# NeRdTheNed/deft4j

Measured on NVIDIA B200. Metric: input MB/s optimised (-m NONE), higher is better.
Workload: dtype u8

## Files before the change

deft4j_b200/csrc/engine.cuh:

```cuda
#pragma once
#include "enum.cuh"
#include "parse.cuh"

namespace d4 {

#ifndef D4_ENG_NT
#define D4_ENG_NT 256
#endif
#ifndef D4_ENG_MINB
#define D4_ENG_MINB 4
#endif
constexpr int ENG_NT = D4_ENG_NT;
constexpr int ENG_NW = ENG_NT / 32;
constexpr int ERR_TREE = 11, ERR_ROUNDS = 12, ERR_WRITER = 2, ERR_POOL = 15, ERR_INTERNAL = 16;

__device__ long long* g_trace = nullptr;
__device__ unsigned g_trace_cap = 0;
__device__ unsigned g_trace_n = 0;

struct Cand {
    Tab tab;
    Hdr hdr;
    long long payload;
    uint16_t mid, tabid;
    uint32_t pad2;
};
__device__ __forceinline__ long long cand_size(const Cand& c) { return c.payload + (c.tab.type == 2 ? c.hdr.bits : 0); }

struct BlkView {
    const uint32_t* sym;
    const uint32_t* symout;
    const uint8_t* out;
    uint32_t n;
    uint32_t nwords;
    uint64_t ulen;
    uint64_t out_off;
};

constexpr int DC_TILE = 512;
constexpr int DCN = 16;
constexpr int LCN = 12;
constexpr int MAXLIT = 64;
constexpr int WS_BYTES = 3072;
#ifndef D4_HQS
#define D4_HQS 4608
#endif
constexpr int HQS = D4_HQS, HQL = 1024;
constexpr int SLOT_B = MAXM, SLOT_BEST = MAXM + 1;
static_assert(DC_TILE == 32 * 16 && DC_TILE > 258, "a tile is one warp-wide 128-bit load and no match spans more than two tiles");

#ifdef D4_PROF
__device__ unsigned long long g_prof[64];
#define P0() const long long p0_ = clock64()
#define P1(cat) do { if (threadIdx.x == 0) { atomicAdd(&g_prof[cat], (unsigned long long)(clock64() - p0_)); atomicAdd(&g_prof[32 + (cat)], 1ull); } } while (0)
#define PCOUNT(cat, k) do { if (threadIdx.x == 0) atomicAdd(&g_prof[32 + (cat)], (unsigned long long)(k)); } while (0)
#else
#define P0()
#define P1(cat)
#define PCOUNT(cat, k)
#endif
enum { PR_BLOCK = 0, PR_ROUND, PR_SWEEP, PR_SELECT, PR_PASS, PR_DC, PR_RECODE, PR_TREES, PR_HDR_DEFAULT, PR_HDROP, PR_TRIALS,
       PR_LOAD, PR_MATERIAL, PR_REBASE, PR_INTERN_MASK, PR_INTERN_TAB, PR_FIXED, PR_SLOWTREE, PR_SEGMENTED, PR_HIST,
       PR_PASS_MAIN, PR_PASS_HQ, PR_LEAST_APPLY, PR_PASS_LEAST, PR_MASKS };

struct EngSmem {
    SymState sym;
// ... 16 lines not shown
    int sweepOk[4], segImproved, segmentedRound;
    struct { long long bestSize, restMin; SC best; unsigned bestIndex, candIndex; int bestStored, bestArg; } carry;
    unsigned char tabDc[MAXT];
    unsigned short dcOwner[DCN];
    int dcNext;
    unsigned char tabLit[MAXT];
    unsigned long long litHash[MAXLIT];
    unsigned short litRep[MAXLIT];
    unsigned char litSlot[MAXLIT];
    unsigned char slotLit[LCN];
    int nLit, litNext;
    uint32_t ctab[256];
    uint8_t refL[32], refD[32];
    union alignas(16) {
        unsigned char ws[ENG_NW][WS_BYTES];
        uint32_t P[ENG_NW][DC_TILE + 4 + 36];
        struct { Tab tab; Hdr hdr; TreeWsCL ws; } mat;
        struct { uint32_t nS, nL; uint32_t qs[HQS]; uint32_t ql[HQL]; } hq;
    } u;
};

__shared__ EngSmem g_es;
#define ES (&g_es)

struct EngScratch {
    unsigned char* slab;
    size_t stride;
    size_t oMasks;
    size_t oTabs;
    size_t oHdrs;
    size_t oHists;
    size_t oTabHash;
    size_t oDc;
    size_t oKd;
    size_t oMinfo;
    size_t oTileFirst;
    size_t oTrialAll;
    size_t oRecs;
    size_t oSlowWs;
    size_t oPerm;
    size_t oDcBits;
    size_t oItems;
    uint32_t maxwords, maxtiles;
};
inline size_t eng_scratch_layout(EngScratch& sc, uint32_t maxwords, uint64_t maxu) {
    sc.maxwords = maxwords;
    sc.maxtiles = (uint32_t)(maxu / DC_TILE + 4);
    const size_t maxn = (size_t)maxwords * 32;
    size_t o = 0;
    auto take = [&](size_t bytes) { const size_t at = o; o = (o + bytes + 255) & ~(size_t)255; return at; };
    sc.oRecs = take(2 * sizeof(Cand));
    sc.oTabHash = take(sizeof(unsigned long long) * MAXT);
    sc.oTabs = take(sizeof(Tab) * (MAXT + ENG_NW));
    sc.oTileFirst = take(4 * (size_t)sc.maxtiles);
    sc.oMinfo = take(4 * maxn);
    sc.oPerm = take(4 * maxn);
    sc.oItems = take(4 * ((size_t)maxwords + 64));
    sc.oDc = take(2 * maxn * LCN);
    sc.oKd = take(2 * maxn);
    sc.oDcBits = take(4 * (size_t)maxwords * 2 * DCN);
    sc.oMasks = take(4 * (size_t)(MAXM + 2) * maxwords);
    sc.oHists = take(4 * (size_t)(MAXM + 2) * 320);
    sc.oHdrs = take(sizeof(Hdr) * MAXH);
    sc.oTrialAll = take(4 * (size_t)MAXT * 56);
    sc.oSlowWs = take(sizeof(TreeWs<290, 584>) * ENG_NW);
    sc.stride = (o + ((size_t)2 << 20) - 1) & ~(((size_t)2 << 20) - 1);
    return sc.stride;
}

struct Eng {
    static constexpr short DC_BLOCKED = 0x7FFF, DC_NOT_MATCH = 0x7FFE;
    BlkView v;
    uint32_t* masks;
    uint32_t maxwords, maxn;
    Tab* tabs;
    Hdr* hdrs;
    uint32_t* hists;
    unsigned long long* tabHash;
    short* dc;
    uint16_t* kd;
    uint32_t* minfo;
    uint32_t* tileFirst;
    int* trialAll;
    Cand* recs;
    TreeWs<290, 584>* slowWs;
    uint32_t* perm;
    uint32_t* dcBits;
    uint32_t* items;
    int tid;
    bool bigWeights;

    __device__ uint32_t* maskp(int id) const { return masks + (size_t)id * maxwords; }
    __device__ uint32_t* histp(int id) const { return hists + (size_t)id * 320; }

    __device__ __noinline__ unsigned long long hash_words(const uint32_t* p, int nwords32) {
        unsigned long long h = 0;
#pragma unroll 1
        for (int k = tid; k < nwords32; k += ENG_NT) {
            unsigned long long x = (unsigned long long)p[k] + 0x9E3779B97F4A7C15ull * (unsigned long long)(k + 1);
            x ^= x >> 30; x *= 0xBF58476D1CE4E5B9ull; x ^= x >> 27; x *= 0x94D049BB133111EBull; x ^= x >> 31;
            h += x;
        }
#pragma unroll 1
        for (int d = 16; d > 0; d >>= 1) h += __shfl_xor_sync(0xffffffffu, h, d);
        if ((tid & 31) == 0) ES->hred[tid >> 5] = h;
        __syncthreads();
        unsigned long long r = 0;
#pragma unroll 1
        for (int k = 0; k < ENG_NW; k++) r += ES->hred[k];
        __syncthreads();
        return r | 1ull;
    }
    static __device__ __forceinline__ unsigned long long hash_words_warp(const uint32_t* p, int nwords32, int lane) {
        unsigned long long h = 0;
// ... 69 lines not shown
    }

    __device__ __noinline__ int intern_mask(unsigned long long h) {
        P0();
        const int fresh = ES->sym.nMasks;
        const uint32_t* q = maskp(fresh);
        __syncthreads();
        if (tid == 0) { ES->tmpIdx = -1; ES->redAny2 = 0; }
        __syncthreads();
#pragma unroll 1
        for (int k = tid; k < fresh; k += ENG_NT)
            if (ES->maskHash[k] == h) atomicMax(&ES->tmpIdx, k);
        __syncthreads();
        int hit = ES->tmpIdx;
        if (hit >= 0) {
            const uint32_t* a = maskp(hit);
            bool diff = false;
#pragma unroll 1
            for (uint32_t k = tid; k < v.nwords; k += ENG_NT) diff |= a[k] != q[k];
            if (diff) ES->redAny2 = 1;
            __syncthreads();
            if (ES->redAny2) hit = -1;
        }
        __syncthreads();
        if (hit < 0) {
            hit = fresh;
            if (tid == 0) { ES->maskHash[fresh] = h; ES->sym.rc[fresh].state = ST_EMPTY; ES->sym.nMasks = fresh + 1; }
        }
        __syncthreads();
        P1(PR_INTERN_MASK);
        return hit;
    }

    __device__ __noinline__ void build_views() {
        const uint32_t a0 = (uint32_t)(v.out_off & ~15ull);
        const uint32_t ntiles = (uint32_t)(((v.out_off - a0) + v.ulen) / DC_TILE) + 2;
#pragma unroll 1
        for (uint32_t t = tid; t < ntiles; t += ENG_NT) tileFirst[t] = v.n;
        __syncthreads();
#pragma unroll 1
        for (uint32_t i = tid; i < v.n; i += ENG_NT) {
            const uint32_t s = v.sym[i];
            const uint32_t rel = v.symout[i] - a0;
            const bool mt = sym_is_match(s);
            const uint32_t kq = mt ? (uint32_t)(sym_lensym(s) - 256) : 0u;
            const uint32_t dsy = mt ? (uint32_t)dist_sym(sym_dist(s)) : 0u;
            minfo[i] = mt ? ((s & 0x1FF) | (dsy << 9) | (kq << 14) | ((rel & (DC_TILE - 1)) << 19)) : 0u;
            kd[i] = (uint16_t)(kq | (dsy << 5));
            const uint32_t ti = rel / DC_TILE;
            const int tprev = i ? (int)((v.symout[i - 1] - a0) / DC_TILE) : -1;
            if ((int)ti != tprev) tileFirst[ti] = i;
        }
        if (tid < 32) ES->leastCnt[tid] = 0;
        __syncthreads();
#pragma unroll 1
        for (uint32_t i = tid; i < v.n; i += ENG_NT) { const uint32_t s = v.sym[i]; if (sym_is_match(s)) atomicAdd(&ES->leastCnt[sym_lensym(s) - 257], 1); }
        __syncthreads();
        if (tid == 0) {
            uint32_t acc = 0;
#pragma unroll 1
            for (int b = 0; b < 32; b++) { ES->binStart[b] = acc; acc += (uint32_t)ES->leastCnt[b]; ES->leastCnt[b] = (int)ES->binStart[b]; }
            ES->binStart[32] = acc;
        }
        __syncthreads();
        if (tid == 0) {
            uint32_t acc = 0;
#pragma unroll 1
            for (int b = 0; b < 32; b++) { ES->itemStart[b] = acc; acc += (ES->binStart[b + 1] - ES->binStart[b] + 31) / 32; }
            ES->itemStart[32] = acc;
        }
#pragma unroll 1
        for (uint32_t i = tid; i < v.n; i += ENG_NT) {
            const uint32_t s = v.sym[i];
            if (sym_is_match(s)) perm[atomicAdd(&ES->leastCnt[sym_lensym(s) - 257], 1)] = i;
        }
        __syncthreads();
        if (tid < 32) {
            uint32_t o = ES->itemStart[tid];
#pragma unroll 1
            for (uint32_t j = ES->binStart[tid]; j < ES->binStart[tid + 1]; j += 32) items[o++] = j | ((uint32_t)tid << 27);
        }
#pragma unroll 1
        for (uint32_t i = v.n + tid; i < v.nwords * 32; i += ENG_NT) {
            minfo[i] = 0; kd[i] = 0;
        }
        __syncthreads();
    }

    __device__ __noinline__ void pass_hist_full(int mid) {
        P0();
        const uint32_t* m = maskp(mid);
#pragma unroll 1
        for (int k = tid; k < 320; k += ENG_NT) ES->hist[k] = 0;
        __syncthreads();
#pragma unroll 1
        for (uint32_t i = tid; i < v.n; i += ENG_NT) {
            uint32_t s = v.sym[i];
            if (!sym_is_match(s)) {
                if (s <= 256) atomicAdd(&ES->hist[s], 1u);
            } else if (!((m[i >> 5] >> (i & 31)) & 1)) {
                atomicAdd(&ES->hist[sym_lensym(s)], 1u);
                atomicAdd(&ES->hist[288 + dist_sym(sym_dist(s))], 1u);
            } else {
                const uint8_t* p = v.out + v.symout[i];
                int len = sym_len(s);
#pragma unroll 1
                for (int k = 0; k < len; k++) atomicAdd(&ES->hist[p[k]], 1u);
            }
        }
        __syncthreads();
        P1(PR_HIST);
    }

    __device__ __noinline__ long long hist_payload(const uint32_t* h, const Tab& t) {
        long long acc = 0;
#pragma unroll 1
        for (int k = tid; k < 318; k += ENG_NT) {
            const uint32_t f = h[k];
            if (!f) continue;
            int bits;
            if (k < 257) bits = t.L[k];
            else if (k < 286) bits = t.L[k] + len_ebits_of(k);
            else if (k >= 288) bits = t.D[k - 288] + dist_ebits_of(k - 288);
            else bits = 0;
            acc += (long long)f * bits;
        }
        if (tid == 0) ES->red = 0;
        __syncthreads();
#pragma unroll 1
        for (int d = 16; d > 0; d >>= 1) acc += __shfl_xor_sync(0xffffffffu, acc, d);
        if ((tid & 31) == 0 && acc) atomicAdd(&ES->red, (unsigned long long)acc);
        __syncthreads();
        const long long r = (long long)ES->red;
        __syncthreads();
        return r;
    }

    __device__ __noinline__ void reset_pools() {
// ... 30 lines not shown
        if (tid == 0) { ES->maskHash[0] = h; ES->sym.nMasks = 1; }
        const Cand& src = recs[0];
        SC b;
        b.mid = 0; b.ok = 1; b.hid = -1; b.tabid = TAB_FIXED; b.type = 1;
        long long pay = src.payload;
        if (toFixed) pay = hist_payload(h0, tabs[TAB_FIXED]);
        else if (src.tab.type == 2) {
            uint32_t* st = (uint32_t*)&tabs[MAXT];
            const uint32_t* q = (const uint32_t*)&src.tab;
#pragma unroll 1
            for (int k = tid; k < (int)(sizeof(Tab) / 4); k += ENG_NT) st[k] = q[k];
            uint32_t* hd = (uint32_t*)&hdrs[0];
            const uint32_t* hq = (const uint32_t*)&src.hdr;
#pragma unroll 1
            for (int k = tid; k < (int)(sizeof(Hdr) / 4); k += ENG_NT) hd[k] = hq[k];
            __syncthreads();
            if (tid < 32) {
                const int t = intern_tab_warp(0, tid);
                if (tid == 0) ES->tmpIdx = t;
            }
            __syncthreads();
            b.tabid = (short)ES->tmpIdx; b.type = 2; b.hid = 0;
            if (tid == 0) { ES->sym.hbits[0] = (unsigned short)src.hdr.bits; ES->sym.nHdrs = 1; }
        }
        b.payload = pay;
        if (tid == 0) { ES->en.B = b; ES->en.blockType = b.type; }
        __syncthreads();
    }

    __device__ __noinline__ void load_block(const Cand& src, const uint32_t* maskSrc, bool toFixed) {
        P0();
        __syncthreads();
        bigWeights = v.ulen + (uint64_t)v.n + 4 >= (1ull << 22);
        uint32_t* mb = maskp(SLOT_B);
#pragma unroll 1
        for (uint32_t k = tid; k < v.nwords; k += ENG_NT) mb[k] = maskSrc[k];
        uint32_t* d = (uint32_t*)&recs[0];
        const uint32_t* s = (const uint32_t*)&src;
#pragma unroll 1
        for (int k = tid; k < (int)(sizeof(Cand) / 4); k += ENG_NT) d[k] = s[k];
        build_views();
        pass_hist_full(SLOT_B);
        uint32_t* hb = histp(SLOT_B);
#pragma unroll 1
        for (int k = tid; k < 320; k += ENG_NT) hb[k] = ES->hist[k];
        __syncthreads();
        adopt_B(toFixed);
        if (tid == 0) {
            ES->en.trialAll = trialAll;
            ES->tsink.buf = g_trace; ES->tsink.cap = g_trace_cap; ES->tsink.n = &g_trace_n;
            ES->en.trace = g_trace ? &ES->tsink : nullptr;
            ES->en.storedOK = v.ulen <= 65535;
        }
        __syncthreads();
        P1(PR_LOAD);
    }



    __device__ __forceinline__ void load_ref(int t) {
        const Tab& tb = tabs[t];
        if (tid < 32) ES->refL[tid] = (uint8_t)(tb.L[256 + tid] + (tid > 0 && tid < 30 ? len_ebits_of(256 + tid) : 0));
        else if (tid < 64) ES->refD[tid - 32] = (uint8_t)(tb.D[tid - 32] + (tid - 32 < 30 ? dist_ebits_of(tid - 32) : 0));
    }
    __device__ __forceinline__ int dc_val(const short* lit, uint32_t i) const {
        const int x = lit[i];
        if (x == DC_BLOCKED) return DC_BLOCKED;
        const uint32_t k = kd[i];
        return x - ES->refL[k & 31] - ES->refD[k >> 5];
    }

    __device__ __noinline__ const short* ensure_lit(int t) {
        int ls = ES->tabLit[t];
        if (ls == 0xFF) {
            __syncthreads();
            const uint32_t* q = (const uint32_t*)tabs[t].L;
            unsigned long long hh = 0;
            if (tid < 64) {
                unsigned long long x = (unsigned long long)q[tid] + 0x9E3779B97F4A7C15ull * (unsigned long long)(tid + 1);
                x ^= x >> 30; x *= 0xBF58476D1CE4E5B9ull; x ^= x >> 27; x *= 0x94D049BB133111EBull; x ^= x >> 31;
                hh = x;
            }
            const unsigned long long h = cta_sum64(hh);
            if (tid == 0) ES->tmpIdx = -1;
            __syncthreads();
            const int nl = ES->nLit;
#pragma unroll 1
            for (int k = 0; k < nl; k++) {
                if (ES->litHash[k] != h) continue;
                const uint32_t* r = (const uint32_t*)tabs[ES->litRep[k]].L;
                const int diff = __syncthreads_or(tid < 64 && r[tid] != q[tid]);
                if (!diff) { if (tid == 0) ES->tmpIdx = k; break; }
            }
            __syncthreads();
            if (tid == 0) {
                int k = ES->tmpIdx;
                if (k < 0) {
                    if (ES->nLit == MAXLIT) {
                        ES->nLit = 0;
                        for (int j = 0; j < MAXT; j++) ES->tabLit[j] = 0xFF;
                        for (int j = 0; j < LCN; j++) ES->slotLit[j] = 0xFF;
                    }
// ... 132 lines not shown
                    carryPart = __shfl_sync(0xffffffffu, nPart, src);
                    carryEnd = __shfl_sync(0xffffffffu, nEnd, src);
                }
            }
            __syncwarp();
        }
#undef D4_DC_ONE
#undef D4_PFX
        __syncthreads();
        P1(PR_DC);
        return d;
    }

    __device__ __noinline__ const uint32_t* ensure_masks(int t, const short* lit) {
        load_ref(t);
        int slot = ES->tabDc[t];
        __syncthreads();
        if (slot != 0xFF) return dcBits + (size_t)slot * 2 * maxwords;
        P0();
        if (tid == 0) {
            slot = ES->dcNext;
            ES->dcNext = (slot + 1) % DCN;
            const int owner = ES->dcOwner[slot];
            if (owner != 0xFFFF) ES->tabDc[owner] = 0xFF;
            ES->dcOwner[slot] = (unsigned short)t;
            ES->tabDc[t] = (unsigned char)slot;
            ES->tmpIdx = slot;
        }
        __syncthreads();
        slot = ES->tmpIdx;
        uint32_t* negW = dcBits + (size_t)slot * 2 * maxwords;
        uint8_t* negB = (uint8_t*)negW;
        uint8_t* zerB = (uint8_t*)(negW + maxwords);
        const uint32_t end = v.nwords * 32;
        uint32_t i0 = (uint32_t)tid * 8;
        uint4 lq = make_uint4(0, 0, 0, 0), kq = lq;
        if (i0 < end) { kq = *(const uint4*)(kd + i0); lq = *(const uint4*)(lit + i0); }
#pragma unroll 1
        while (i0 < end) {
            const uint4 cl = lq, ck = kq;
            const uint32_t nx = i0 + ENG_NT * 8;
            if (nx < end) { kq = *(const uint4*)(kd + nx); lq = *(const uint4*)(lit + nx); }
            uint32_t nb = 0, zb = 0;
            if (ck.x | ck.y | ck.z | ck.w) {
                const uint32_t lw[4] = {cl.x, cl.y, cl.z, cl.w}, kw[4] = {ck.x, ck.y, ck.z, ck.w};
#pragma unroll
                for (int u = 0; u < 8; u++) {
                    const uint32_t k = (u & 1) ? (kw[u >> 1] >> 16) : (kw[u >> 1] & 0xffffu);
                    const int x = (int)(short)((u & 1) ? (lw[u >> 1] >> 16) : (lw[u >> 1] & 0xffffu));
                    if (k && x != DC_BLOCKED) {
                        const int val = x - ES->refL[k & 31] - ES->refD[k >> 5];
                        nb |= (val < 0 ? 1u : 0u) << u;
                        zb |= (val == 0 ? 1u : 0u) << u;
                    }
                }
            }
            negB[i0 >> 3] = (uint8_t)nb;
            zerB[i0 >> 3] = (uint8_t)zb;
            i0 = nx;
        }
        __syncthreads();
        P1(PR_MASKS);
        return negW;
    }

    __device__ __noinline__ void hist_delta_replace(uint32_t i) {
        const uint32_t s = v.sym[i];
        atomicSub(&ES->hist[sym_lensym(s)], 1u);
        atomicSub(&ES->hist[288 + dist_sym(sym_dist(s))], 1u);
        const uint8_t* p = v.out + v.symout[i];
        const int len = sym_len(s);
#pragma unroll 1
        for (int k = 0; k < len; k++) atomicAdd(&ES->hist[p[k]], 1u);
    }
    __device__ __noinline__ void hq_push_warp(uint32_t nbits, uint32_t i0, int lane) {
        const uint32_t cnt = (uint32_t)__popc(nbits);
        uint32_t incl = cnt;
#pragma unroll
        for (int dd = 1; dd < 32; dd <<= 1) { const uint32_t y = __shfl_up_sync(0xffffffffu, incl, dd); if (lane >= dd) incl += y; }
        const uint32_t total = __shfl_sync(0xffffffffu, incl, 31);
        if (!total) return;
        uint32_t base = 0;
        if (lane == 0) base = atomicAdd(&ES->u.hq.nS, total);
        base = __shfl_sync(0xffffffffu, base, 0) + incl - cnt;
#pragma unroll 1
        for (uint32_t b = nbits; b; b &= b - 1, base++) {
            const uint32_t i = i0 + (uint32_t)__ffs((int)b) - 1;
            if (base < HQS) ES->u.hq.qs[base] = i;
            else {
                hist_delta_replace(i);
                if (ES->hqLit) atomicAdd(&ES->red, (unsigned long long)(long long)(-dc_val(ES->hqLit, i)));
            }
        }
    }
    __device__ __noinline__ void hq_apply(const short* lit) {
        __syncthreads();
        const uint32_t nS = min(ES->u.hq.nS, (uint32_t)HQS);
        long long sv = 0;
#pragma unroll 1
        for (uint32_t j = tid; j < nS; j += ENG_NT) {
            const uint32_t i = ES->u.hq.qs[j];
            const uint32_t mi = minfo[i];
            const uint32_t so = v.symout[i];
            if (lit) sv -= dc_val(lit, i);
            const int len = (int)(mi & 0x1FF) + 3;
            atomicSub(&ES->hist[256 + ((mi >> 14) & 31)], 1u);
            atomicSub(&ES->hist[288 + ((mi >> 9) & 31)], 1u);
            if (len > 24) {
                const uint32_t k = atomicAdd(&ES->u.hq.nL, 1u);
                if (k < HQL) { ES->u.hq.ql[k] = i; continue; }
            }
            const uint8_t* p = v.out + so;
#pragma unroll 1
            for (int k = 0; k < len; k += 8) {
                uint32_t b[8];
#pragma unroll
                for (int q = 0; q < 8; q++) b[q] = (k + q < len) ? (uint32_t)p[k + q] : 256u;
#pragma unroll
                for (int q = 0; q < 8; q++) if (b[q] < 256u) atomicAdd(&ES->hist[b[q]], 1u);
            }
        }
        if (lit) {
#pragma unroll
            for (int dd = 16; dd > 0; dd >>= 1) sv += __shfl_xor_sync(0xffffffffu, sv, dd);
            if ((tid & 31) == 0 && sv) atomicAdd(&ES->red, (unsigned long long)sv);
        }
        __syncthreads();
        const uint32_t nL = min(ES->u.hq.nL, (uint32_t)HQL);
        const int lane = tid & 31;
#pragma unroll 1
        for (uint32_t j = (uint32_t)(tid >> 5); j < nL; j += ENG_NW) {
            const uint32_t i = ES->u.hq.ql[j];
            const int len = (int)(minfo[i] & 0x1FF) + 3;
            const uint8_t* p = v.out + v.symout[i];
#pragma unroll 1
            for (int k = lane; k < len; k += 32) atomicAdd(&ES->hist[p[k]], 1u);
        }
        __syncthreads();
    }
    __device__ __forceinline__ void hist_store_delta(int dst, int src) {
        const uint32_t* hs = histp(src);
        uint32_t* hd = histp(dst);
#pragma unroll 1
        for (int k = tid; k < 320; k += ENG_NT) hd[k] = hs[k] + ES->hist[k];
    }

    __device__ __noinline__ void pass_replace(int slot, int mid, int tabid, bool prune) {
        if (ES->sym.nMasks >= MAXM) { if (tid == 0) ES->sym.overflow = 1; __syncthreads(); return; }
        const short* d = ensure_lit(tabid);
        const uint32_t* negW = ensure_masks(tabid, d);
        const uint32_t* zerW = negW + maxwords;
        P0();
#pragma unroll 1
        for (int k = tid; k < 320; k += ENG_NT) ES->hist[k] = 0;
        if (tid == 0) { ES->red = 0; ES->redAny = 0; ES->u.hq.nS = 0; ES->u.hq.nL = 0; ES->hqLit = d; }
        __syncthreads();
        const int fresh = ES->sym.nMasks;
        const uint32_t* mo = maskp(mid);
        uint32_t* mn = maskp(fresh);
        unsigned long long hsh = 0;
        const int lane = tid & 31;
        bool any = false;
#pragma unroll 1
        for (uint32_t kb = (uint32_t)(tid & ~31); kb < v.nwords; kb += ENG_NT) {
            const uint32_t k = kb + (uint32_t)lane;
            uint32_t cand = 0;
            if (k < v.nwords) {
// ... 26 lines not shown
            if (prune && ES->sym.rc[newmid].state == ST_EMPTY) ES->sym.rc[newmid].state = ST_PENDING;
        }
        __syncthreads();
    }

    __device__ __noinline__ void pass_least(int slot0, int slot1, int mid, int tabid) {
        if (ES->sym.nMasks + 2 > MAXM) { if (tid == 0) ES->sym.overflow = 1; __syncthreads(); return; }
        const short* d = ensure_lit(tabid);
        load_ref(tabid);
        P0();
        if (tid < 32) { ES->leastSum[tid] = 0; ES->leastCnt[tid] = 0; }
        if (tid == 0) { ES->leastBlocked = 0; ES->leastSeen = 0; }
        __syncthreads();
        const int lane = tid & 31;
        const uint8_t* mbytes = (const uint8_t*)maskp(mid);
        {
            const uint32_t nItems = ES->itemStart[32];
#pragma unroll 1
            for (uint32_t it = tid; it < nItems; it += ENG_NT) {
                const uint32_t w = items[it];
                const int bin = (int)(w >> 27);
                uint32_t j = w & 0x7FFFFFFu;
                const uint32_t jend = min(ES->binStart[bin + 1], j + 32);
                int sum = 0, cnt = 0;
                bool blocked = false, seen = false;
#pragma unroll 1
                for (; j < jend; j += 8) {
                    uint32_t idx[8];
                    int xv[8];
                    uint32_t mk[8];
#pragma unroll
                    for (int u = 0; u < 8; u++) idx[u] = j + u < jend ? perm[j + u] : 0u;
#pragma unroll
                    for (int u = 0; u < 8; u++) { xv[u] = d[idx[u]]; mk[u] = mbytes[idx[u] >> 3] | ((uint32_t)kd[idx[u]] << 8); }
#pragma unroll
                    for (int u = 0; u < 8; u++) {
                        const bool live = j + u < jend && !((mk[u] >> (idx[u] & 7)) & 1);
                        seen |= live;
                        const bool blk = live && xv[u] == DC_BLOCKED;
                        blocked |= blk;
                        if (live && !blk) { sum += xv[u] - ES->refL[bin + 1] - ES->refD[mk[u] >> 13]; cnt++; }
                    }
                }
                if (seen) atomicOr(&ES->leastSeen, 1u << bin);
                if (blocked) atomicOr(&ES->leastBlocked, 1u << bin);
                if (cnt) { atomicAdd(&ES->leastSum[bin], sum); atomicAdd(&ES->leastCnt[bin], cnt); }
            }
        }
        __syncthreads();
        if (tid == 0) {
#pragma unroll 1
            for (int mode = 0; mode < 2; mode++) {
                int rem = -1, remSize = 0, remFreq = 0;
#pragma unroll 1
                for (int i = 0; i < 32; i++) {
                    if (!((ES->leastBlocked >> i) & 1) && ((ES->leastSeen >> i) & 1)) {
                        bool doRem = mode == 1 ? ES->leastCnt[i] < remFreq : ES->leastSum[i] < remSize;
                        if (rem == -1 || doRem) { rem = i; remSize = ES->leastSum[i]; remFreq = ES->leastCnt[i]; }
                    }
                }
                ES->leastRem[mode] = rem; ES->leastSize[mode] = remSize;
            }
        }
        __syncthreads();
        P1(PR_PASS_LEAST);
        int doneMid = -1, doneRem = -2;
#pragma unroll 1
        for (int mode = 0; mode < 2; mode++) {
            const int slot = mode ? slot1 : slot0;
            if (slot < 0) continue;
            const int rem = ES->leastRem[mode];
            int newmid = mid;
            if (rem >= 0 && rem == doneRem) newmid = doneMid;
            else if (rem >= 0) {
// ... 678 lines not shown
                const uint32_t* hs = (const uint32_t*)&recs[0].hdr;
                uint32_t* hd = (uint32_t*)&hdrs[hid];
#pragma unroll 1
                for (int k = tid; k < (int)(sizeof(Hdr) / 4); k += ENG_NT) hd[k] = hs[k];
                __syncthreads();
                if (tid == 0) {
                    ES->sym.hbits[hid] = (unsigned short)recs[0].hdr.bits;
                    ES->sym.nHdrs = hid + 1;
                    ES->sym.hop[hid][0] = ES->sym.hop[hid][1] = ES->sym.hop[hid][2] = 0;
                }
                b.hid = (short)hid;
            }
            __syncthreads();
            if (tid == 0) { ES->en.B = b; ES->en.blockType = b.type; }
            __syncthreads();
        } else {
            adopt_B(false);
        }
        P1(PR_REBASE);
    }
};

__device__ inline void eng_init(Eng& e, const EngScratch& sc, int cta) {
    e.tid = (int)threadIdx.x;
    e.maxwords = sc.maxwords;
    e.maxn = sc.maxwords * 32;
    unsigned char* base = sc.slab + (size_t)cta * sc.stride;
    e.masks = reinterpret_cast<uint32_t*>(base + sc.oMasks);
    e.tabs = reinterpret_cast<Tab*>(base + sc.oTabs);
    e.hdrs = reinterpret_cast<Hdr*>(base + sc.oHdrs);
    e.hists = reinterpret_cast<uint32_t*>(base + sc.oHists);
    e.tabHash = reinterpret_cast<unsigned long long*>(base + sc.oTabHash);
    e.dc = reinterpret_cast<short*>(base + sc.oDc);
    e.kd = reinterpret_cast<uint16_t*>(base + sc.oKd);
    e.minfo = reinterpret_cast<uint32_t*>(base + sc.oMinfo);
    e.tileFirst = reinterpret_cast<uint32_t*>(base + sc.oTileFirst);
    e.trialAll = reinterpret_cast<int*>(base + sc.oTrialAll);
    e.recs = reinterpret_cast<Cand*>(base + sc.oRecs);
    e.slowWs = reinterpret_cast<TreeWs<290, 584>*>(base + sc.oSlowWs);
    e.perm = reinterpret_cast<uint32_t*>(base + sc.oPerm);
    e.dcBits = reinterpret_cast<uint32_t*>(base + sc.oDcBits);
    e.items = reinterpret_cast<uint32_t*>(base + sc.oItems);
    e.bigWeights = false;
    if (threadIdx.x == 0) ES->err = 0;
    __syncthreads();
}

}
```

deft4j_b200/csrc/optimise.cuh:

```cuda
#pragma once
#include "engine.cuh"

namespace d4 {

constexpr int MAXR = 64;

struct BlkState {
    Cand cand;
    uint64_t sym_off;
    uint64_t out_off;
    uint64_t mask_off;
    uint64_t out_len;
    uint32_t n_sym;
    int32_t alive;
    int32_t bfinal;
    int32_t nrounds;
    uint64_t bit_pos;
    long long size_bits;
};
struct RoundRec { long long sizeI, sizeC1, restMin, best; };
struct RoundLog { RoundRec r[MAXR]; };

struct StreamState {
    uint64_t blk_base;
// ... 13 lines not shown
__device__ __forceinline__ long long blk_size(const BlkState& b, long long alignment) {
    return b.cand.tab.type == 0 ? stored_size(b.out_len, alignment) : cand_size(b.cand);
}

__global__ void k_init_state(const BlockRec* __restrict__ recs, const uint64_t* __restrict__ mask_offs,
                             BlkState* __restrict__ bs, uint64_t nblk) {
    uint64_t i = (uint64_t)blockIdx.x * blockDim.x + threadIdx.x;
    if (i >= nblk) return;
    const BlockRec& r = recs[i];
    BlkState& b = bs[i];
    b.cand.tab = r.tab;
    b.cand.tab.type = r.type;
    b.cand.tab.pad[0] = b.cand.tab.pad[1] = b.cand.tab.pad[2] = 0;
    b.cand.hdr = r.hdr;
    b.cand.payload = r.payload_bits;
    b.sym_off = r.sym_base;
    b.out_off = r.out_base;
    b.mask_off = mask_offs[i];
    b.out_len = r.out_len;
    b.n_sym = r.n_sym;
    b.alive = 1;
    b.bfinal = r.bfinal;
    b.nrounds = 0;
    b.bit_pos = r.hdr_bit;
    b.size_bits = (long long)(r.end_bit - r.hdr_bit) - 3;
}

__device__ inline void eng_view(Eng& e, const BlkState& b, const uint32_t* sym, const uint32_t* symout, const uint8_t* out,
                                uint32_t n, uint64_t ulen) {
    e.v.sym = sym + b.sym_off;
    e.v.symout = symout + b.sym_off;
    e.v.out = out;
    e.v.n = n;
    e.v.nwords = (n + 31) / 32;
    e.v.ulen = ulen;
    e.v.out_off = b.out_off;
}

__global__ void __launch_bounds__(ENG_NT, D4_ENG_MINB)
k_opt_blocks(const uint32_t* __restrict__ jobs, uint32_t njobs, BlkState* __restrict__ bs, RoundLog* __restrict__ logs,
             const uint32_t* __restrict__ sym, const uint32_t* __restrict__ symout, const uint8_t* __restrict__ out,
             uint32_t* __restrict__ maskpool, EngScratch sc, unsigned* __restrict__ counter, int* __restrict__ gerr) {
    EngSmem& S = g_es;
    __shared__ uint32_t s_job;
    Eng e;
    eng_init(e, sc, blockIdx.x);
    const int tid = threadIdx.x;
    while (true) {
        if (tid == 0) s_job = atomicAdd(counter, 1u);
        __syncthreads();
        const uint32_t job = s_job;
        __syncthreads();
        if (job >= njobs) break;
        P0();
        BlkState& b = bs[jobs[job]];
        eng_view(e, b, sym, symout, out, b.n_sym, b.out_len);
        e.load_block(b.cand, maskpool + b.mask_off, false);
        RoundLog& lg = logs[jobs[job]];
        int r = 0;
        long long prevBest = -1;
        while (true) {
            e.optimise_block(-1);
            if (S.err) break;
            if (tid == 0 && r < MAXR) {
                RoundRec rr; rr.sizeI = S.en.sizeI; rr.sizeC1 = S.en.sizeC1; rr.restMin = S.en.restMin; rr.best = S.en.bestSize;
                lg.r[r] = rr;
            }
            const bool improved = S.en.bestSize < S.en.sizeI;
            bool bad = prevBest >= 0 && S.en.sizeI != prevBest;
            int badWhat = 1;
            __syncthreads();
            if (improved) {
                e.pass_hist_full(SLOT_BEST);
                const long long truePay = e.hist_payload(S.hist, e.recs[1].tab);
                if (truePay != e.recs[1].payload) { bad = true; badWhat = 2; }
                if (cand_size(e.recs[1]) != S.en.bestSize) { bad = true; badWhat = 3; }
            }
            if (bad && tid == 0) {
                if (atomicMax(gerr, 13) < 13) {
                    gerr[1] = (int)jobs[job]; gerr[2] = r; gerr[3] = (int)S.en.bestIndex;
                    gerr[4] = (int)S.en.bestSize; gerr[5] = (int)cand_size(e.recs[1]); gerr[6] = badWhat; gerr[7] = (int)prevBest;
                }
            }
            __syncthreads();
            prevBest = S.en.bestSize;
            r++;
            if (!improved) break;
            if (r >= MAXR) { if (tid == 0) S.err = ERR_ROUNDS; break; }
            e.advance_to_best();
        }
        __syncthreads();
        if (r > 1 && !S.err) {
            const uint32_t* s = (const uint32_t*)&e.recs[0];
            uint32_t* d = (uint32_t*)&b.cand;
            for (int k = tid; k < (int)(sizeof(Cand) / 4); k += ENG_NT) d[k] = s[k];
            const uint32_t* m = e.maskp(SLOT_B);
            uint32_t* pm = maskpool + b.mask_off;
            for (uint32_t k = tid; k < e.v.nwords; k += ENG_NT) pm[k] = m[k];
        }
        if (tid == 0) b.nrounds = r;
        __syncthreads();
        if (S.err) { if (tid == 0) { atomicMax(gerr, S.err); S.err = 0; } }
        __syncthreads();
        P1(PR_BLOCK);
    }
}

__device__ void finish_stream(EngSmem& S, Eng& e, StreamState& st, BlkState* __restrict__ bs, const RoundLog* __restrict__ logs,
                              uint32_t* __restrict__ sym, const uint32_t* __restrict__ symout, const uint8_t* __restrict__ out,
                              uint32_t* __restrict__ maskpool, int merge, int* __restrict__ gerr) {
    __shared__ long long s_pos, s_saved;
    __shared__ int s_cur, s_next, s_do, s_first;
    if (!st.selected || st.status != ST_OK) return;
    const int tid = threadIdx.x;
    BlkState* B = bs + st.blk_base;
    const uint32_t nb = st.n_blocks;

    {
        constexpr int RT = 64, RR = 4;
        struct Tile { unsigned long long out_len[RT]; int type[RT]; RoundRec rr[RT][RR]; };
        static_assert(sizeof(Tile) <= sizeof(EngSmem), "replay tile must fit in the engine's shared storage");
        Tile& T = *reinterpret_cast<Tile*>(&S);
        __shared__ long long s_rpos, s_rsaved;
        __shared__ int s_stop;
        __shared__ uint32_t s_first_alive, s_n_alive;
        if (tid == 0) { s_rpos = 0; s_rsaved = 0; s_stop = 0; s_first_alive = nb; s_n_alive = 0; }
        __syncthreads();
        {
            uint32_t fa = nb, na = 0;
            for (uint32_t k = tid; k < nb; k += ENG_NT) if (B[k].alive) { if (fa == nb) fa = k; na++; }
            if (na) { atomicMin(&s_first_alive, fa); atomicAdd(&s_n_alive, na); }
// ... 92 lines not shown
                                long long mergedSize = stored_size(c.out_len + nx.out_len, s_pos);
                                long long cs = curSize + 3 + nextSize - mergedSize;
                                if (cs > 0) {
                                    s_saved += cs;
                                    c.out_len += nx.out_len;
                                    c.n_sym = 0;
                                    nx.alive = 0;
                                    s_do = 2;
                                }
                            }
                        } else if (nx.cand.tab.type != 0) {
                            s_do = 1;
                        }
                    }
                    if (s_do == 0) s_do = 3;
                    if (s_do != 1) s_pos += blk_size(c, s_pos);
                } else {
                    s_saved += blk_size(c, s_pos + 3) + 3;
                    c.alive = 0;
                    s_do = 4;
                }
            }
            __syncthreads();
            int action = s_do;
            if (action == 1) {
                BlkState& c = B[cur];
                BlkState& nx = B[s_next];
                const uint32_t nA = c.n_sym, nB = nx.n_sym;
                const uint32_t gap = (uint32_t)(nx.sym_off - c.sym_off), span = gap + nB;
                if (tid == 0) sym[c.sym_off + nA - 1] = SYM_NOP;
                eng_view(e, c, sym, symout, out, span, c.out_len + nx.out_len);
                {
                    uint32_t* m = e.maskp(SLOT_BEST);
                    for (uint32_t k = tid; k < e.v.nwords; k += ENG_NT) m[k] = 0;
                    __syncthreads();
                    const uint32_t* ma = maskpool + c.mask_off;
                    const uint32_t* mb = maskpool + nx.mask_off;
                    for (uint32_t i = tid; i < nA; i += ENG_NT)
                        if ((ma[i >> 5] >> (i & 31)) & 1) atomicOr(&m[i >> 5], 1u << (i & 31));
                    for (uint32_t i = tid; i < nB; i += ENG_NT)
                        if ((mb[i >> 5] >> (i & 31)) & 1) atomicOr(&m[(gap + i) >> 5], 1u << ((gap + i) & 31));
                    __syncthreads();
                    e.load_block(c.cand, m, true);
                }
                const long long pos = s_pos;
                e.optimise_block(stored_size(e.v.ulen, pos));
                if (tid == 0) {
                    long long curSize = blk_size(c, pos);
                    long long nextSize = blk_size(nx, pos + curSize + 3);
                    long long cs = curSize + 3 + nextSize - S.en.bestSize;
                    s_do = cs > 0 ? 5 : 6;
                    if (cs > 0) s_saved += cs;
                }
                __syncthreads();
                if (s_do == 5) {
                    if (!S.en.bestStored) {
                        const uint32_t* s = (const uint32_t*)&e.recs[1];
                        uint32_t* d = (uint32_t*)&c.cand;
                        for (int k = tid; k < (int)(sizeof(Cand) / 4); k += ENG_NT) d[k] = s[k];
                        const uint32_t* bm = e.maskp(SLOT_BEST);
                        uint32_t* pm = maskpool + c.mask_off;
                        for (uint32_t k = tid; k < e.v.nwords; k += ENG_NT) pm[k] = bm[k];
                    }
                    __syncthreads();
                    if (tid == 0) {
                        if (S.en.bestStored) c.cand.tab.type = 0;
                        c.n_sym = span;
                        c.out_len += nx.out_len;
                        nx.alive = 0;
                    }
                } else {
                    if (tid == 0) sym[c.sym_off + nA - 1] = 256;
                }
                __syncthreads();
                if (tid == 0) s_pos += blk_size(c, s_pos);
                action = (s_do == 5) ? 2 : 3;
                __syncthreads();
            }
            if (action == 4) break;
            if (tid == 0) {
                if (action == 3) {
                    s_cur = s_next < 0 ? (int)nb : s_next;
                    s_first = 0;
                }
            }
            __syncthreads();
        }
        if (S.err && tid == 0) { atomicMax(gerr, S.err); S.err = 0; }
    }
    __syncthreads();

    {
        constexpr int LT = 128;
        struct LTile { unsigned long long out_len[LT], bit_pos[LT]; long long csize[LT], size_bits[LT]; int type[LT], alive[LT]; };
        static_assert(sizeof(LTile) <= sizeof(EngSmem), "layout tile must fit in the engine's shared storage");
// ... 63 lines not shown
```

Measured before the change: 1168.

## Compact engine views to match-only index space with rank-mapped masks

Rebuilds the engine's per-block views so that minfo, output offsets, perm, tile index and masks are indexed only over match symbols, using ballot flags and per-word prefix ranks. The per-literal histogram is computed once and cached, so later passes walk only matches. Masks are translated between the full-symbol pool format and the compacted format on load and store. This shrinks the work and memory traffic in every hist, delta-cost and mask pass, at the cost of extra bit-scatter and gather steps and more complex indexing.

New measurement: 1335, median of 6. +14.3%, better.

```diff
diff --git a/deft4j_b200/csrc/engine.cuh b/deft4j_b200/csrc/engine.cuh
--- a/deft4j_b200/csrc/engine.cuh
+++ b/deft4j_b200/csrc/engine.cuh
@@ -32,6 +32,7 @@
     const uint32_t* symout;
     const uint8_t* out;
     uint32_t n;
+    uint32_t nm;
     uint32_t nwords;
     uint64_t ulen;
     uint64_t out_off;
@@ -114,8 +115,11 @@
     size_t oHists;
     size_t oTabHash;
     size_t oDc;
-    size_t oKd;
     size_t oMinfo;
+    size_t oMout;
+    size_t oMflag;
+    size_t oMrank;
+    size_t oLitHist;
     size_t oTileFirst;
     size_t oTrialAll;
     size_t oRecs;
@@ -134,12 +138,15 @@
     sc.oRecs = take(2 * sizeof(Cand));
     sc.oTabHash = take(sizeof(unsigned long long) * MAXT);
     sc.oTabs = take(sizeof(Tab) * (MAXT + ENG_NW));
+    sc.oLitHist = take(4 * 320);
+    sc.oMflag = take(4 * (size_t)maxwords);
+    sc.oMrank = take(4 * (size_t)maxwords);
     sc.oTileFirst = take(4 * (size_t)sc.maxtiles);
     sc.oMinfo = take(4 * maxn);
+    sc.oMout = take(4 * maxn);
     sc.oPerm = take(4 * maxn);
     sc.oItems = take(4 * ((size_t)maxwords + 64));
     sc.oDc = take(2 * maxn * LCN);
-    sc.oKd = take(2 * maxn);
     sc.oDcBits = take(4 * (size_t)maxwords * 2 * DCN);
     sc.oMasks = take(4 * (size_t)(MAXM + 2) * maxwords);
     sc.oHists = take(4 * (size_t)(MAXM + 2) * 320);
@@ -151,7 +158,7 @@
 }
 
 struct Eng {
-    static constexpr short DC_BLOCKED = 0x7FFF, DC_NOT_MATCH = 0x7FFE;
+    static constexpr short DC_BLOCKED = 0x7FFF;
     BlkView v;
     uint32_t* masks;
     uint32_t maxwords, maxn;
@@ -160,8 +167,11 @@
     uint32_t* hists;
     unsigned long long* tabHash;
     short* dc;
-    uint16_t* kd;
     uint32_t* minfo;
+    uint32_t* mout;
+    uint32_t* mflag;
+    uint32_t* mrank;
+    uint32_t* litHist;
     uint32_t* tileFirst;
     int* trialAll;
     Cand* recs;
@@ -297,78 +307,141 @@
         return hit;
     }
 
+    __device__ __forceinline__ uint32_t sym_words() const { return (v.n + 31) / 32; }
+
     __device__ __noinline__ void build_views() {
+        const int lane = tid & 31, wid = tid >> 5;
+        const uint32_t nsw = sym_words();
+#pragma unroll 1
+        for (uint32_t k = (uint32_t)wid; k < nsw; k += ENG_NW) {
+            const uint32_t i = 32 * k + (uint32_t)lane;
+            const uint32_t f = __ballot_sync(0xffffffffu, i < v.n && sym_is_match(v.sym[i]));
+            if (lane == 0) mflag[k] = f;
+        }
+#pragma unroll 1
+        for (int k = tid; k < 320; k += ENG_NT) ES->hist[k] = 0;
+        if (tid < 32) ES->leastCnt[tid] = 0;
+        __syncthreads();
+        {
+            const uint32_t per = (nsw + ENG_NT - 1) / ENG_NT;
+            const uint32_t k0 = min(nsw, (uint32_t)tid * per), k1 = min(nsw, k0 + per);
+            uint32_t c = 0;
+#pragma unroll 1
+            for (uint32_t k = k0; k < k1; k++) c += (uint32_t)__popc(mflag[k]);
+            uint32_t incl = c;
+#pragma unroll
+            for (int dd = 1; dd < 32; dd <<= 1) { const uint32_t y = __shfl_up_sync(0xffffffffu, incl, dd); if (lane >= dd) incl += y; }
+            if (lane == 31) ES->wt[wid] = incl;
+            __syncthreads();
+            uint32_t base = incl - c, total = 0;
+#pragma unroll 1
+            for (int w = 0; w < ENG_NW; w++) { const uint32_t x = ES->wt[w]; if (w < wid) base += x; total += x; }
+#pragma unroll 1
+            for (uint32_t k = k0; k < k1; k++) { mrank[k] = base; base += (uint32_t)__popc(mflag[k]); }
+            v.nm = total;
+            v.nwords = (total + 31) / 32;
+        }
+        __syncthreads();
         const uint32_t a0 = (uint32_t)(v.out_off & ~15ull);
+#pragma unroll 1
+        for (uint32_t k = (uint32_t)wid; k < nsw; k += ENG_NW) {
+            const uint32_t i = 32 * k + (uint32_t)lane;
+            if (i >= v.n) continue;
+            const uint32_t f = mflag[k];
+            const uint32_t s = v.sym[i];
+            if ((f >> lane) & 1) {
+                const uint32_t j = mrank[k] + (uint32_t)__popc(f & ((1u << lane) - 1u));
+                const uint32_t so = v.symout[i];
+                const uint32_t kq = (uint32_t)(sym_lensym(s) - 256), dsy = (uint32_t)dist_sym(sym_dist(s));
+                minfo[j] = (s & 0x1FF) | (dsy << 9) | (kq << 14) | (((so - a0) & (DC_TILE - 1)) << 19);
+                mout[j] = so;
+                atomicAdd(&ES->leastCnt[kq - 1], 1);
+            } else if (s <= 256) atomicAdd(&ES->hist[s], 1u);
+        }
         const uint32_t ntiles = (uint32_t)(((v.out_off - a0) + v.ulen) / DC_TILE) + 2;
 #pragma unroll 1
-        for (uint32_t t = tid; t < ntiles; t += ENG_NT) tileFirst[t] = v.n;
-        __syncthreads();
-#pragma unroll 1
-        for (uint32_t i = tid; i < v.n; i += ENG_NT) {
-            const uint32_t s = v.sym[i];
-            const uint32_t rel = v.symout[i] - a0;
-            const bool mt = sym_is_match(s);
-            const uint32_t kq = mt ? (uint32_t)(sym_lensym(s) - 256) : 0u;
-            const uint32_t dsy = mt ? (uint32_t)dist_sym(sym_dist(s)) : 0u;
-            minfo[i] = mt ? ((s & 0x1FF) | (dsy << 9) | (kq << 14) | ((rel & (DC_TILE - 1)) << 19)) : 0u;
-            kd[i] = (uint16_t)(kq | (dsy << 5));
-            const uint32_t ti = rel / DC_TILE;
-            const int tprev = i ? (int)((v.symout[i - 1] - a0) / DC_TILE) : -1;
-            if ((int)ti != tprev) tileFirst[ti] = i;
-        }
-        if (tid < 32) ES->leastCnt[tid] = 0;
-        __syncthreads();
-#pragma unroll 1
-        for (uint32_t i = tid; i < v.n; i += ENG_NT) { const uint32_t s = v.sym[i]; if (sym_is_match(s)) atomicAdd(&ES->leastCnt[sym_lensym(s) - 257], 1); }
-        __syncthreads();
+        for (uint32_t t = tid; t < ntiles; t += ENG_NT) tileFirst[t] = v.nm;
+        __syncthreads();
+#pragma unroll 1
+        for (int k = tid; k < 320; k += ENG_NT) litHist[k] = ES->hist[k];
+#pragma unroll 1
+        for (uint32_t j = tid; j < v.nm; j += ENG_NT) {
+            const uint32_t ti = (mout[j] - a0) / DC_TILE;
+            const uint32_t t0 = j ? (mout[j - 1] - a0) / DC_TILE + 1 : 0u;
+#pragma unroll 1
+            for (uint32_t t = t0; t <= ti; t++) tileFirst[t] = j;
+        }
         if (tid == 0) {
             uint32_t acc = 0;
 #pragma unroll 1
             for (int b = 0; b < 32; b++) { ES->binStart[b] = acc; acc += (uint32_t)ES->leastCnt[b]; ES->leastCnt[b] = (int)ES->binStart[b]; }
             ES->binStart[32] = acc;
-        }
-        __syncthreads();
-        if (tid == 0) {
-            uint32_t acc = 0;
+            acc = 0;
 #pragma unroll 1
             for (int b = 0; b < 32; b++) { ES->itemStart[b] = acc; acc += (ES->binStart[b + 1] - ES->binStart[b] + 31) / 32; }
             ES->itemStart[32] = acc;
         }
-#pragma unroll 1
-        for (uint32_t i = tid; i < v.n; i += ENG_NT) {
-            const uint32_t s = v.sym[i];
-            if (sym_is_match(s)) perm[atomicAdd(&ES->leastCnt[sym_lensym(s) - 257], 1)] = i;
-        }
-        __syncthreads();
+        __syncthreads();
+#pragma unroll 1
+        for (uint32_t j = tid; j < v.nm; j += ENG_NT) perm[atomicAdd(&ES->leastCnt[((minfo[j] >> 14) & 31) - 1], 1)] = j;
         if (tid < 32) {
             uint32_t o = ES->itemStart[tid];
 #pragma unroll 1
             for (uint32_t j = ES->binStart[tid]; j < ES->binStart[tid + 1]; j += 32) items[o++] = j | ((uint32_t)tid << 27);
         }
-#pragma unroll 1
-        for (uint32_t i = v.n + tid; i < v.nwords * 32; i += ENG_NT) {
-            minfo[i] = 0; kd[i] = 0;
-        }
-        __syncthreads();
+        __syncthreads();
+    }
+
+    __device__ __noinline__ void load_mask(const uint32_t* src, int slot) {
+        uint32_t* md = maskp(slot);
+#pragma unroll 1
+        for (uint32_t k = tid; k < v.nwords; k += ENG_NT) md[k] = 0;
+        __syncthreads();
+#pragma unroll 1
+        for (uint32_t k = tid; k < sym_words(); k += ENG_NT) {
+            const uint32_t m = src[k];
+            uint32_t f = mflag[k];
+            if (!(m & f)) continue;
+            uint32_t x = 0;
+#pragma unroll 1
+            for (int c = 0; f; f &= f - 1, c++) x |= ((m >> (__ffs((int)f) - 1)) & 1u) << c;
+            const uint32_t r = mrank[k], sh = r & 31;
+            atomicOr(&md[r >> 5], x << sh);
+            if (sh && (x >> (32 - sh))) atomicOr(&md[(r >> 5) + 1], x >> (32 - sh));
+        }
+        __syncthreads();
+    }
+    __device__ __noinline__ void store_mask(int slot, uint32_t* dst) {
+        const uint32_t* ms = maskp(slot);
+#pragma unroll 1
+        for (uint32_t k = tid; k < sym_words(); k += ENG_NT) {
+            uint32_t f = mflag[k], out = 0;
+            if (f) {
+                const uint32_t r = mrank[k], sh = r & 31, w = r >> 5;
+                uint32_t x = ms[w] >> sh;
+                if (sh && w + 1 < v.nwords) x |= ms[w + 1] << (32 - sh);
+#pragma unroll 1
+                for (int c = 0; f; f &= f - 1, c++) out |= ((x >> c) & 1u) << (__ffs((int)f) - 1);
+            }
+            dst[k] = out;
+        }
     }
 
     __device__ __noinline__ void pass_hist_full(int mid) {
         P0();
         const uint32_t* m = maskp(mid);
 #pragma unroll 1
-        for (int k = tid; k < 320; k += ENG_NT) ES->hist[k] = 0;
-        __syncthreads();
-#pragma unroll 1
-        for (uint32_t i = tid; i < v.n; i += ENG_NT) {
-            uint32_t s = v.sym[i];
-            if (!sym_is_match(s)) {
-                if (s <= 256) atomicAdd(&ES->hist[s], 1u);
-            } else if (!((m[i >> 5] >> (i & 31)) & 1)) {
-                atomicAdd(&ES->hist[sym_lensym(s)], 1u);
-                atomicAdd(&ES->hist[288 + dist_sym(sym_dist(s))], 1u);
+        for (int k = tid; k < 320; k += ENG_NT) ES->hist[k] = litHist[k];
+        __syncthreads();
+#pragma unroll 1
+        for (uint32_t j = tid; j < v.nm; j += ENG_NT) {
+            const uint32_t mi = minfo[j];
+            if (!((m[j >> 5] >> (j & 31)) & 1)) {
+                atomicAdd(&ES->hist[256 + ((mi >> 14) & 31)], 1u);
+                atomicAdd(&ES->hist[288 + ((mi >> 9) & 31)], 1u);
             } else {
-                const uint8_t* p = v.out + v.symout[i];
-                int len = sym_len(s);
+                const uint8_t* p = v.out + mout[j];
+                const int len = (int)(mi & 0x1FF) + 3;
 #pragma unroll 1
                 for (int k = 0; k < len; k++) atomicAdd(&ES->hist[p[k]], 1u);
             }
@@ -465,14 +538,12 @@
         P0();
         __syncthreads();
         bigWeights = v.ulen + (uint64_t)v.n + 4 >= (1ull << 22);
-        uint32_t* mb = maskp(SLOT_B);
-#pragma unroll 1
-        for (uint32_t k = tid; k < v.nwords; k += ENG_NT) mb[k] = maskSrc[k];
         uint32_t* d = (uint32_t*)&recs[0];
         const uint32_t* s = (const uint32_t*)&src;
 #pragma unroll 1
         for (int k = tid; k < (int)(sizeof(Cand) / 4); k += ENG_NT) d[k] = s[k];
         build_views();
+        load_mask(maskSrc, SLOT_B);
         pass_hist_full(SLOT_B);
         uint32_t* hb = histp(SLOT_B);
 #pragma unroll 1
@@ -496,11 +567,11 @@
         if (tid < 32) ES->refL[tid] = (uint8_t)(tb.L[256 + tid] + (tid > 0 && tid < 30 ? len_ebits_of(256 + tid) : 0));
         else if (tid < 64) ES->refD[tid - 32] = (uint8_t)(tb.D[tid - 32] + (tid - 32 < 30 ? dist_ebits_of(tid - 32) : 0));
     }
-    __device__ __forceinline__ int dc_val(const short* lit, uint32_t i) const {
-        const int x = lit[i];
+    __device__ __forceinline__ int dc_val(const short* lit, uint32_t j) const {
+        const int x = lit[j];
         if (x == DC_BLOCKED) return DC_BLOCKED;
-        const uint32_t k = kd[i];
-        return x - ES->refL[k & 31] - ES->refD[k >> 5];
+        const uint32_t mi = minfo[j];
+        return x - ES->refL[(mi >> 14) & 31] - ES->refD[(mi >> 9) & 31];
     }
 
     __device__ __noinline__ const short* ensure_lit(int t) {
@@ -699,44 +770,43 @@
         uint32_t* negW = dcBits + (size_t)slot * 2 * maxwords;
         uint8_t* negB = (uint8_t*)negW;
         uint8_t* zerB = (uint8_t*)(negW + maxwords);
-        const uint32_t end = v.nwords * 32;
-        uint32_t i0 = (uint32_t)tid * 8;
-        uint4 lq = make_uint4(0, 0, 0, 0), kq = lq;
-        if (i0 < end) { kq = *(const uint4*)(kd + i0); lq = *(const uint4*)(lit + i0); }
-#pragma unroll 1
-        while (i0 < end) {
-            const uint4 cl = lq, ck = kq;
-            const uint32_t nx = i0 + ENG_NT * 8;
-            if (nx < end) { kq = *(const uint4*)(kd + nx); lq = *(const uint4*)(lit + nx); }
+        const uint32_t end = v.nwords * 32, nm = v.nm;
+        uint32_t j0 = (uint32_t)tid * 8;
+        uint4 lq = make_uint4(0, 0, 0, 0), mq0 = lq, mq1 = lq;
+        if (j0 < nm) { lq = *(const uint4*)(lit + j0); mq0 = *(const uint4*)(minfo + j0); mq1 = *(const uint4*)(minfo + j0 + 4); }
+#pragma unroll 1
+        while (j0 < end) {
+            const uint4 cl = lq, c0 = mq0, c1 = mq1;
+            const uint32_t nx = j0 + ENG_NT * 8;
+            if (nx < nm) { lq = *(const uint4*)(lit + nx); mq0 = *(const uint4*)(minfo + nx); mq1 = *(const uint4*)(minfo + nx + 4); }
             uint32_t nb = 0, zb = 0;
-            if (ck.x | ck.y | ck.z | ck.w) {
-                const uint32_t lw[4] = {cl.x, cl.y, cl.z, cl.w}, kw[4] = {ck.x, ck.y, ck.z, ck.w};
+            if (j0 < nm) {
+                const uint32_t lw[4] = {cl.x, cl.y, cl.z, cl.w}, mw[8] = {c0.x, c0.y, c0.z, c0.w, c1.x, c1.y, c1.z, c1.w};
 #pragma unroll
                 for (int u = 0; u < 8; u++) {
-                    const uint32_t k = (u & 1) ? (kw[u >> 1] >> 16) : (kw[u >> 1] & 0xffffu);
                     const int x = (int)(short)((u & 1) ? (lw[u >> 1] >> 16) : (lw[u >> 1] & 0xffffu));
-                    if (k && x != DC_BLOCKED) {
-                        const int val = x - ES->refL[k & 31] - ES->refD[k >> 5];
+                    if (j0 + u < nm && x != DC_BLOCKED) {
+                        const int val = x - ES->refL[(mw[u] >> 14) & 31] - ES->refD[(mw[u] >> 9) & 31];
                         nb |= (val < 0 ? 1u : 0u) << u;
                         zb |= (val == 0 ? 1u : 0u) << u;
                     }
                 }
             }
-            negB[i0 >> 3] = (uint8_t)nb;
-            zerB[i0 >> 3] = (uint8_t)zb;
-            i0 = nx;
+            negB[j0 >> 3] = (uint8_t)nb;
+            zerB[j0 >> 3] = (uint8_t)zb;
+            j0 = nx;
         }
         __syncthreads();
         P1(PR_MASKS);
         return negW;
     }
 
-    __device__ __noinline__ void hist_delta_replace(uint32_t i) {
-        const uint32_t s = v.sym[i];
-        atomicSub(&ES->hist[sym_lensym(s)], 1u);
-        atomicSub(&ES->hist[288 + dist_sym(sym_dist(s))], 1u);
-        const uint8_t* p = v.out + v.symout[i];
-        const int len = sym_len(s);
+    __device__ __noinline__ void hist_delta_replace(uint32_t j) {
+        const uint32_t mi = minfo[j];
+        atomicSub(&ES->hist[256 + ((mi >> 14) & 31)], 1u);
+        atomicSub(&ES->hist[288 + ((mi >> 9) & 31)], 1u);
+        const uint8_t* p = v.out + mout[j];
+        const int len = (int)(mi & 0x1FF) + 3;
 #pragma unroll 1
         for (int k = 0; k < len; k++) atomicAdd(&ES->hist[p[k]], 1u);
     }
@@ -768,7 +838,7 @@
         for (uint32_t j = tid; j < nS; j += ENG_NT) {
             const uint32_t i = ES->u.hq.qs[j];
             const uint32_t mi = minfo[i];
-            const uint32_t so = v.symout[i];
+            const uint32_t so = mout[i];
             if (lit) sv -= dc_val(lit, i);
             const int len = (int)(mi & 0x1FF) + 3;
             atomicSub(&ES->hist[256 + ((mi >> 14) & 31)], 1u);
@@ -799,7 +869,7 @@
         for (uint32_t j = (uint32_t)(tid >> 5); j < nL; j += ENG_NW) {
             const uint32_t i = ES->u.hq.ql[j];
             const int len = (int)(minfo[i] & 0x1FF) + 3;
-            const uint8_t* p = v.out + v.symout[i];
+            const uint8_t* p = v.out + mout[i];
 #pragma unroll 1
             for (int k = lane; k < len; k += 32) atomicAdd(&ES->hist[p[k]], 1u);
         }
@@ -892,14 +962,14 @@
 #pragma unroll
                     for (int u = 0; u < 8; u++) idx[u] = j + u < jend ? perm[j + u] : 0u;
 #pragma unroll
-                    for (int u = 0; u < 8; u++) { xv[u] = d[idx[u]]; mk[u] = mbytes[idx[u] >> 3] | ((uint32_t)kd[idx[u]] << 8); }
+                    for (int u = 0; u < 8; u++) { xv[u] = d[idx[u]]; mk[u] = mbytes[idx[u] >> 3] | (minfo[idx[u]] & (31u << 9)); }
 #pragma unroll
                     for (int u = 0; u < 8; u++) {
                         const bool live = j + u < jend && !((mk[u] >> (idx[u] & 7)) & 1);
                         seen |= live;
                         const bool blk = live && xv[u] == DC_BLOCKED;
                         blocked |= blk;
-                        if (live && !blk) { sum += xv[u] - ES->refL[bin + 1] - ES->refD[mk[u] >> 13]; cnt++; }
+                        if (live && !blk) { sum += xv[u] - ES->refL[bin + 1] - ES->refD[mk[u] >> 9]; cnt++; }
                     }
                 }
                 if (seen) atomicOr(&ES->leastSeen, 1u << bin);
@@ -1644,8 +1714,11 @@
     e.hists = reinterpret_cast<uint32_t*>(base + sc.oHists);
     e.tabHash = reinterpret_cast<unsigned long long*>(base + sc.oTabHash);
     e.dc = reinterpret_cast<short*>(base + sc.oDc);
-    e.kd = reinterpret_cast<uint16_t*>(base + sc.oKd);
     e.minfo = reinterpret_cast<uint32_t*>(base + sc.oMinfo);
+    e.mout = reinterpret_cast<uint32_t*>(base + sc.oMout);
+    e.mflag = reinterpret_cast<uint32_t*>(base + sc.oMflag);
+    e.mrank = reinterpret_cast<uint32_t*>(base + sc.oMrank);
+    e.litHist = reinterpret_cast<uint32_t*>(base + sc.oLitHist);
     e.tileFirst = reinterpret_cast<uint32_t*>(base + sc.oTileFirst);
     e.trialAll = reinterpret_cast<int*>(base + sc.oTrialAll);
     e.recs = reinterpret_cast<Cand*>(base + sc.oRecs);
diff --git a/deft4j_b200/csrc/optimise.cuh b/deft4j_b200/csrc/optimise.cuh
--- a/deft4j_b200/csrc/optimise.cuh
+++ b/deft4j_b200/csrc/optimise.cuh
@@ -69,7 +69,8 @@
     e.v.symout = symout + b.sym_off;
     e.v.out = out;
     e.v.n = n;
-    e.v.nwords = (n + 31) / 32;
+    e.v.nm = 0;
+    e.v.nwords = 0;
     e.v.ulen = ulen;
     e.v.out_off = b.out_off;
 }
@@ -131,9 +132,7 @@
             const uint32_t* s = (const uint32_t*)&e.recs[0];
             uint32_t* d = (uint32_t*)&b.cand;
             for (int k = tid; k < (int)(sizeof(Cand) / 4); k += ENG_NT) d[k] = s[k];
-            const uint32_t* m = e.maskp(SLOT_B);
-            uint32_t* pm = maskpool + b.mask_off;
-            for (uint32_t k = tid; k < e.v.nwords; k += ENG_NT) pm[k] = m[k];
+            e.store_mask(SLOT_B, maskpool + b.mask_off);
         }
         if (tid == 0) b.nrounds = r;
         __syncthreads();
@@ -292,7 +291,7 @@
                 eng_view(e, c, sym, symout, out, span, c.out_len + nx.out_len);
                 {
                     uint32_t* m = e.maskp(SLOT_BEST);
-                    for (uint32_t k = tid; k < e.v.nwords; k += ENG_NT) m[k] = 0;
+                    for (uint32_t k = tid; k < e.sym_words(); k += ENG_NT) m[k] = 0;
                     __syncthreads();
                     const uint32_t* ma = maskpool + c.mask_off;
                     const uint32_t* mb = maskpool + nx.mask_off;
@@ -318,9 +317,7 @@
                         const uint32_t* s = (const uint32_t*)&e.recs[1];
                         uint32_t* d = (uint32_t*)&c.cand;
                         for (int k = tid; k < (int)(sizeof(Cand) / 4); k += ENG_NT) d[k] = s[k];
-                        const uint32_t* bm = e.maskp(SLOT_BEST);
-                        uint32_t* pm = maskpool + c.mask_off;
-                        for (uint32_t k = tid; k < e.v.nwords; k += ENG_NT) pm[k] = bm[k];
+                        e.store_mask(SLOT_BEST, maskpool + c.mask_off);
                     }
                     __syncthreads();
                     if (tid == 0) {
```
